# georgegrosu1/torch-admm-deconv

Measured on AMD Instinct MI355X. Metric: ADMM iterations/sec, batch-64 1024x1024x3, 50 iters; rel-L2 vs CPU ref, higher is better.
Workload: dtype f32

## Files before the change

torch-admm-deconv_amd/csrc/admm_capi.hip:

```cpp
#include <hip/hip_runtime.h>

#include <cstdlib>
#include <cstring>
#include <mutex>
#include <string>
#include <type_traits>
#include <vector>

#include "gcol_mm.hpp"
#include "knobs.hpp"
#include "mixed_capi.hpp"
#include "odd_capi.hpp"
#include "state_kernels.hpp"
#include "admm_tv.h"

using namespace admm;

namespace {

thread_local std::string g_err;

int fail(int code, const std::string& msg) {
    g_err = msg;
    return code;
// ... 319 lines not shown
            hipLaunchKernelGGL((k_iso_norm<N, true, false, true>), dim3(nb), dim3(G::NT), G::lds_bytes(), s, a);
        else if (first)
            hipLaunchKernelGGL((k_iso_norm<N, true, false, false>), dim3(nb), dim3(G::NT), G::lds_bytes(), s, a);
        else if (hist)
            hipLaunchKernelGGL((k_iso_norm<N, false, true, false>), dim3(nb), dim3(G::NT), G::lds_bytes(), s, a);
        else if (pl)
            hipLaunchKernelGGL((k_iso_norm<N, false, false, true>), dim3(nb), dim3(G::NT), G::lds_bytes(), s, a);
        else
            hipLaunchKernelGGL((k_iso_norm<N, false, false, false>), dim3(nb), dim3(G::NT), G::lds_bytes(), s, a);
        return launch_check("k_iso_norm");
    }
    template <bool ISO, bool LASTK, bool FIRSTK> static void bpa(const BwdArgs& a, unsigned nb, hipStream_t s) {
        using BG = BwdGeom<N>;
        hipLaunchKernelGGL((k_bwd_pass_a<N, ISO, LASTK, FIRSTK>), dim3(nb), dim3(BG::NT), BG::lds_bytes(), s, a);
    }
    static int bwd_pass_a(const BwdArgs& a, bool iso, bool lastk, bool firstk, hipStream_t s) {
        const unsigned nb = (unsigned)((a.nstrips + BwdGeom<N>::SG - 1) / BwdGeom<N>::SG);
        const int sel = (iso ? 4 : 0) | (lastk ? 2 : 0) | (firstk ? 1 : 0);
        switch (sel) {
            case 0: bpa<false, false, false>(a, nb, s); break;
            case 1: bpa<false, false, true>(a, nb, s); break;
            case 2: bpa<false, true, false>(a, nb, s); break;
            case 3: bpa<false, true, true>(a, nb, s); break;
            case 4: bpa<true, false, false>(a, nb, s); break;
            case 5: bpa<true, false, true>(a, nb, s); break;
            case 6: bpa<true, true, false>(a, nb, s); break;
            default: bpa<true, true, true>(a, nb, s); break;
        }
        return launch_check("k_bwd_pass_a");
    }
    static int bwd_iso_q(const BwdIsoArgs& a, bool lastk, hipStream_t s) {
        const unsigned nb = blocks(a.nitems);
        if (lastk)
            hipLaunchKernelGGL((k_bwd_iso_q<N, true>), dim3(nb), dim3(G::NT), G::lds_bytes(), s, a);
        else
            hipLaunchKernelGGL((k_bwd_iso_q<N, false>), dim3(nb), dim3(G::NT), G::lds_bytes(), s, a);
        return launch_check("k_bwd_iso_q");
    }
};

template <class F> int with_row(int N, F&& f) {
    switch (N) {
        case 8: return f(RowOps<8>{});
        case 16: return f(RowOps<16>{});
        case 32: return f(RowOps<32>{});
        case 64: return f(RowOps<64>{});
        case 128: return f(RowOps<128>{});
        case 256: return f(RowOps<256>{});
        case 512: return f(RowOps<512>{});
        case 1024: return f(RowOps<1024>{});
        default: return fail(ADMM_TV_EUNSUPPORTED, "unsupported W");
    }
}

template <class F> int with_col(int H, F&& f) {
    switch (H) {
        case 16: return f(std::integral_constant<int, 16>{});
        case 32: return f(std::integral_constant<int, 32>{});
        case 64: return f(std::integral_constant<int, 64>{});
        case 128: return f(std::integral_constant<int, 128>{});
        case 256: return f(std::integral_constant<int, 256>{});
        case 512: return f(std::integral_constant<int, 512>{});
        case 1024: return f(std::integral_constant<int, 1024>{});
        case 2048: return f(std::integral_constant<int, 2048>{});
        case 4096: return f(std::integral_constant<int, 4096>{});
        default: return fail(ADMM_TV_EUNSUPPORTED, "unsupported H");
    }
}

int col_e(int H) { return H >= 1024 ? 16 : H >= 64 ? 8 : 4; }

int passb_order(int H) { return std::max(1, std::min(64, env_int("ADMM_PASSB_GROUP", H >= 1024 ? 2 : 1))); }

int passb_gp(int H, int P, int ppm) {
    (void)H;
    int g = env_int("ADMM_PASSB_GP", 1);
    g = std::max(1, std::min(g, 64));
    while (g > 1 && (ppm % g)) --g;
    (void)P;
    return g;
}

template <int H, int C> int pass_b_hc(const cf* spec, cf* out, const float* fcT, const cf* mT, const cf* twH, int N,
                                      int P, int mode, int ppm, hipStream_t s) {
    using G = ColGeom<H, C>;
    const int colblocks = N / C;
    const int gp = passb_gp(H, P, ppm);
    const dim3 grid((unsigned)((long long)((P + gp - 1) / gp) * colblocks));
    const int order = gp > 1 ? 1 : passb_order(H);
    const int fpack = mode == 0 && env_int("ADMM_PASSB_FPACK", 1) ? 1 : 0;
    const int pmode = env_int("ADMM_PASSB_PMODE", 2);
    if (mode == 0) {
        if (int e = set_lds(k_pass_b<H, C, 0>, G::lds_bytes())) return e;
        hipLaunchKernelGGL((k_pass_b<H, C, 0>), grid, dim3(G::NT), G::lds_bytes(), s, spec, out, fcT, mT, twH, N, colblocks, ppm,
                           order, fpack, gp, P, pmode);
    } else if (mode == 1) {
        if (int e = set_lds(k_pass_b<H, C, 1>, G::lds_bytes())) return e;
        hipLaunchKernelGGL((k_pass_b<H, C, 1>), grid, dim3(G::NT), G::lds_bytes(), s, spec, out, fcT, mT, twH, N, colblocks, ppm,
                           order, fpack, gp, P, pmode);
    } else {
        if (int e = set_lds(k_pass_b<H, C, 2>, G::lds_bytes())) return e;
        hipLaunchKernelGGL((k_pass_b<H, C, 2>), grid, dim3(G::NT), G::lds_bytes(), s, spec, out, fcT, mT, twH, N, colblocks, ppm,
                           order, fpack, gp, P, pmode);
    }
    return launch_check("k_pass_b");
}

template <int H> int pass_b_h(const cf* spec, cf* out, const float* fcT, const cf* mT, const cf* twH, int N, int P,
                              int mode, int ppm, hipStream_t s) {
    constexpr int L = ColGeom<H, 1>::L;
    if constexpr (L <= 64) {
        if (mode == 0 && N >= 16 && env_int("ADMM_PASSB_PAIR", H <= 512 ? 1 : 0)) {
            using G = ColGeom<H, 8>;
            const int colblocks = N / 16;
            if (int e = set_lds(k_pass_b2<H, 8>, G::lds_bytes())) return e;
            hipLaunchKernelGGL((k_pass_b2<H, 8>), dim3((unsigned)((long long)P * colblocks)), dim3(G::NT), G::lds_bytes(),
                               s, spec, out, fcT, twH, N, colblocks, ppm, passb_order(H), env_int("ADMM_PASSB_FPACK", 1) ? 1 : 0);
            return launch_check("k_pass_b2");
        }
        int C = env_int("ADMM_PASSB_C", 8);
        if (C > N) C = N;
        if (C >= 16) return pass_b_hc<H, 16>(spec, out, fcT, mT, twH, N, P, mode, ppm, s);
        return pass_b_hc<H, 8>(spec, out, fcT, mT, twH, N, P, mode, ppm, s);
    } else if constexpr (L == 128) {
        return pass_b_hc<H, 8>(spec, out, fcT, mT, twH, N, P, mode, ppm, s);
    } else {
        return pass_b_hc<H, 4>(spec, out, fcT, mT, twH, N, P, mode, ppm, s);
    }
}

int pass_b_oop(int H, const cf* spec, cf* out, const float* fcT, const cf* mT, const cf* twH, int N, int P, int mode,
               hipStream_t s, int ppm = 0) {
    if (ppm <= 0) ppm = P;
    return with_col(H, [&](auto h) { return pass_b_h<decltype(h)::value>(spec, out, fcT, mT, twH, N, P, mode, ppm, s); });
}

int pass_b(int H, cf* spec, const float* fcT, const cf* mT, const cf* twH, int N, int P, int mode, hipStream_t s,
           int ppm = 0) {
    return pass_b_oop(H, spec, spec, fcT, mT, twH, N, P, mode, s, ppm);
}

template <int H, int C> int xspec_hc(const cf* U, const cf* V, cf* part, const cf* twH, int N, int P, int ppg,
                                     hipStream_t s) {
    using G = ColGeom<H, C>;
    const int colblocks = N / C;
    const int groups = (P + ppg - 1) / ppg;
    if (int e = set_lds(k_xspec<H, C, true>, G::lds_bytes())) return e;
    if (int e = set_lds(k_xspec<H, C, false>, G::lds_bytes())) return e;
    hipLaunchKernelGGL((k_xspec<H, C, true>), dim3(groups), dim3(G::NT), G::lds_bytes(), s, U, V, part, twH, N,
                       colblocks, P, ppg);
    if (colblocks > 1)
        hipLaunchKernelGGL((k_xspec<H, C, false>), dim3(groups * (colblocks - 1)), dim3(G::NT), G::lds_bytes(), s, U,
                           V, part, twH, N, colblocks, P, ppg);
    return launch_check("k_xspec");
}
template <int H> int xspec_h(const cf* U, const cf* V, cf* part, const cf* twH, int N, int P, int ppg, hipStream_t s) {
    constexpr int L = ColGeom<H, 1>::L;
    if constexpr (L <= 64) return xspec_hc<H, 8>(U, V, part, twH, N, P, ppg, s);
    else if constexpr (L == 128) return xspec_hc<H, 8>(U, V, part, twH, N, P, ppg, s);
    else return xspec_hc<H, 4>(U, V, part, twH, N, P, ppg, s);
}
int xspec(int H, const cf* U, const cf* V, cf* part, const cf* twH, int N, int P, int ppg, hipStream_t s) {
    return with_col(H, [&](auto h) { return xspec_h<decltype(h)::value>(U, V, part, twH, N, P, ppg, s); });
}

int grouped_train_check(const admm_tv_desc& d) {
    if (d.groups > 1 && !supported_hw(d.H, d.W))
        return fail(ADMM_TV_EUNSUPPORTED, "grouped training needs power-of-two H, W: one call per module");
    return 0;
}

int validate(const admm_tv_desc* d) {
    if (!d) return fail(ADMM_TV_EINVAL, "null descriptor");
    const bool empty_ok = d->iso && d->allreduce && d->B >= 0 && d->C >= 0;
    if ((empty_ok ? (d->B < 0 || d->C < 0) : (d->B <= 0 || d->C <= 0)) || d->H <= 0 || d->W <= 0 || d->maxit < 0 ||
        d->kh < 0 || d->kw < 0 || d->groups < 0)
        return fail(ADMM_TV_EINVAL, "invalid sizes or maxit");
    if (d->kh != d->kw) return fail(ADMM_TV_ENONSQUARE, "non-square PSF (the reference's H_t swaps H/W pads)");
    if (is_f64(*d) ? !f64_hw(d->H, d->W) : (!supported_hw(d->H, d->W) && !generic_hw(d->H, d->W)))
        return fail(ADMM_TV_EUNSUPPORTED, "unsupported H, W (admm_tv_supported / admm_tv_supported_f64: up to 65,536)");
    if (is_f64(*d) && d->groups > 1) return fail(ADMM_TV_EUNSUPPORTED, "groups > 1: fp32 only");
    if (d->kh > d->H || d->kw > d->W) return fail(ADMM_TV_EKERNEL, "PSF larger than the image");
    if (d->groups > 1 && ((!supported_hw(d->H, d->W) && !mixed_hw(d->H, d->W)) || (d->flags & ADMM_TV_FLAG_PSF_GRAD)))
        return fail(ADMM_TV_EUNSUPPORTED, "groups > 1 needs power-of-two or smooth H, W and no PSF gradient");
    return 0;
}

double spectra_scale(int H, int W) {
    return (supported_hw(H, W) ? 0.5 : 1.0) / ((double)H * (double)W);
}

template <class T>
int setup(const admm_tv_desc& d, const Layout& Lo, void* ws, const T* kern, const T* rho, hipStream_t s) {
    using C = cx_t<T>;
    ProfScope ps(3, s);
    const int H = (int)d.H, W = (int)d.W, N = W / 2, k = d.kh;
    const int nt = 256;
    hipLaunchKernelGGL(k_tables<C>, dim3((std::max(H, W) + nt - 1) / nt), dim3(nt), 0, s, at<C>(ws, Lo.twW),
                       at<C>(ws, Lo.twH), at<double2>(ws, Lo.twHd), H, W);
    if (int e = launch_check("k_tables")) return e;
    if (Lo.gen && !std::is_same<T, double>::value) {
        for (int dim = 0; dim < 2; ++dim) {
            const GPlan pl = make_plan(dim == 0 ? W : H);
            if (pl.ntab == 0) continue;
            hipLaunchKernelGGL(k_blue_tables, dim3((3 * 1024 * 64 + nt - 1) / nt), dim3(nt), 0, s,
                               at<cf>(ws, dim == 0 ? Lo.twW : Lo.twH), pl);
            if (int e = launch_check("k_blue_tables")) return e;
        }
    }
    if (k > 0) {
        const int n = k * (N + 1);
        hipLaunchKernelGGL(k_psf_rows<T>, dim3((n + nt - 1) / nt), dim3(nt), 0, s, kern, at<double2>(ws, Lo.G), k, N, W);
        if (int e = launch_check("k_psf_rows")) return e;
    }
    const int n = (N + 1) * H;
    if (rho) {
        for (int g = 0; g < ngroups_of(d); ++g) {
// ... 918 lines not shown
    const int ns = std::max(1, std::min(kMaxAux + 1, env_setting("ADMM_GEN_STREAMS", 2)));
    const std::vector<long long> parts = gen_parts(P, H, ns);
    const bool glb = make_plan(H, kF64<T>).glb || make_plan(W, kF64<T>).glb;
    if (!d.iso && !train && parts.size() > 1 && !glb && cap == hipStreamCaptureStatusNone) {
        int dev = 0;
        HIPCHK(hipGetDevice(&dev));
        std::vector<hipStream_t> aux;
        for (size_t i = 1; i < parts.size(); ++i) {
            hipStream_t x = aux_stream(s, dev, (int)i - 1);
            if (!x) return fail(ADMM_TV_EHIP, "auxiliary stream");
            aux.push_back(x);
        }
        ForkJoin fj(s, aux);
        if (fj.err != hipSuccess) return fail(ADMM_TV_EHIP, std::string("fork: ") + hipGetErrorString(fj.err));
        int e = 0;
        for (size_t i = 0; i < parts.size() && !e; ++i) {
            const long long p1 = i + 1 < parts.size() ? parts[i + 1] : P;
            e = solve_planes(parts[i], p1 - parts[i], i == 0 ? s : aux[i - 1]);
        }
        const hipError_t je = fj.finish();
        if (e) return e;
        if (je != hipSuccess) return fail(ADMM_TV_EHIP, std::string("join: ") + hipGetErrorString(je));
    } else {
        if (int e = solve_planes(0, P, s)) return e;
    }
    if constexpr (!kF64<T>) {
        if (sout) {
            const int ui = (d.maxit - 1) & 1;
            const bool none = d.maxit == 1 && !sin;
            return state_export(d, Lo, ws, out, none ? nullptr : u[2 * ui], none ? nullptr : u[2 * ui + 1], *sio->out, lam,
                                rho, 0, s);
        }
    }
    return 0;
}

long long mixed_slots(int N) {
    static std::mutex mu;
    static std::vector<std::pair<std::pair<int, int>, long long>> cache;
    int dev = 0;
    if (hipGetDevice(&dev) != hipSuccess) return 512;
    std::lock_guard<std::mutex> lk(mu);
    for (const auto& c : cache)
        if (c.first.first == dev && c.first.second == N) return c.second;
    long long slots = 0;
    int cus = 0;
    if (hipDeviceGetAttribute(&cus, hipDeviceAttributeMultiprocessorCount, dev) == hipSuccess)
        slots = (long long)cus * std::max(1, admm_mixed::pass_a_blocks_per_cu(N));
    if (slots <= 0) return 512;
    cache.push_back({{dev, N}, slots});
    return slots;
}
int strip_rows_mixed(int H, long long rows, int N, long long slots = 0) {
    if (const int e = env_int("ADMM_MIXED_R", 0); e > 0 && H % e == 0) return e;
    const int sg = 256 / std::max(1, admm_mixed::row_lanes(N));
    if (slots <= 0) slots = mixed_slots(N);
    int best = 1;
    double best_t = 1e300;
    for (int R = 1; R <= 32 && R <= H; ++R) {
        if (H % R) continue;
        const long long strips = rows / R;
        const long long blocks = (strips + sg - 1) / sg;
        const double t = (double)((blocks + slots - 1) / slots) * (R + 1);
        if (t < best_t - 1e-9 || (t < best_t + 1e-9 && R > best)) {
            best_t = t;
            best = R;
        }
    }
    return best;
}

struct FusedOps {
    const admm_tv_desc& d;
    const Layout& Lo;
    void* const ws;
    const int H, N;
    cf *const twW, *const twH;
    FusedOps(const admm_tv_desc& d_, const Layout& L, void* w)
        : d(d_), Lo(L), ws(w), H((int)d_.H), N((int)d_.W / 2), twW(at<cf>(w, L.twW)), twH(at<cf>(w, L.twH)) {}
};

struct Pow2Ops : FusedOps {
    static constexpr bool kPsfGrad = true;
    float* const fcT;
    cf* const mT;
    const bool coop;
    const int rev;
    const bool pf;
    Pow2Ops(const admm_tv_desc& d_, const Layout& L, void* w)
        : FusedOps(d_, L, w), fcT(at<float>(w, L.fcT)), mT(at<cf>(w, L.mT)),
          coop(env_int("ADMM_PASSA_COOP", 1) != 0), rev(env_int("ADMM_PASSA_REV", 0)),
          pf(env_int("ADMM_PASSA_PF", 1) != 0) {}
    int modules_per_pass(int G) const { return G; }
    bool lane_paired(bool train) const { return !train && env_int("ADMM_PL", (d.iso || d.W < 1024) ? 1 : 0) != 0; }
    int row_lanes() const {
        int L = 0;
        with_row(N, [&](auto ops) { return L = decltype(ops)::G::L; });
        return L;
    }
    int strip(long long rows, bool aniso_fwd) const { return strip_rows(H, N, rows, aniso_fwd, coop && !rev); }
    int r2c(const float* img, cf* spec, long long rows, hipStream_t s, bool pl = false) const {
        return with_row(N, [&](auto ops) { return decltype(ops)::r2c(img, spec, twW, rows, s, pl); });
    }
    int c2r(const cf* spec, float* img, long long rows, hipStream_t s) const {
        return with_row(N, [&](auto ops) { return decltype(ops)::c2r(spec, img, twW, rows, s); });
    }
    int col(const cf* in, cf* out, long long np, long long ppm, int , hipStream_t s) const {
        return pass_b_oop(H, in, out, fcT, mT, twH, N, (int)np, 0, s, (int)ppm);
    }
    int xspec(const cf* U, const cf* V, cf* part, long long P, int ppg, bool , hipStream_t s) const {
        return ::xspec(H, U, V, part, twH, N, (int)P, ppg, s);
    }
    int iso_norm(const IsoArgs& a, bool first, bool hist, hipStream_t s, bool pl) const {
        return with_row(N, [&](auto ops) { return decltype(ops)::iso_norm(a, first, hist, s, pl); });
    }
    int pass_a(const PassAArgs& a, bool iso, bool first, bool hist, hipStream_t s, bool pl) const {
        return with_row(N, [&](auto ops) { return decltype(ops)::pass_a(a, iso, first, hist, s, pl, coop, pf); });
    }
    int bwd_iso_q(const BwdIsoArgs& a, bool lastk, hipStream_t s) const {
        return with_row(N, [&](auto ops) { return decltype(ops)::bwd_iso_q(a, lastk, s); });
    }
    int bwd_pass_a(const BwdArgs& a, bool iso, bool lastk, bool firstk, hipStream_t s) const {
        return with_row(N, [&](auto ops) { return decltype(ops)::bwd_pass_a(a, iso, lastk, firstk, s); });
    }
    int make_b(const float* xin, float* bb, cf* spec, bool pl, hipStream_t s) const {
        if (d.kh > 0) return psf_transpose_into(d, Lo, ws, xin, bb, spec, 1, s, pl);
        return with_row(N, [&](auto ops) { return decltype(ops)::pair(xin, bb, d.B * d.C * H, s); });
    }
    int apply_ht_t(const float* bbar, float* gxin, cf* spec, hipStream_t s) const {
        return psf_transpose_into(d, Lo, ws, bbar, gxin, spec, 2, s);
    }
};

struct MixedOps : FusedOps {
    static constexpr bool kPsfGrad = true;
    const float* const fcM;
    static constexpr int rev = 0;
    MixedOps(const admm_tv_desc& d_, const Layout& L, void* w) : FusedOps(d_, L, w), fcM(at<float>(w, L.fcM)) {}
    int modules_per_pass(int) const { return 1; }
    bool lane_paired(bool) const { return false; }
    int row_lanes() const { return 0; }
    int strip(long long rows, bool) const { return strip_rows_mixed(H, rows, N); }
    int r2c(const float* img, cf* spec, long long rows, hipStream_t s, bool = false) const {
        return hip_code(admm_mixed::r2c(N, img, spec, twW, rows, s), "k_row_r2c_m");
    }
    int c2r(const cf* spec, float* img, long long rows, hipStream_t s) const {
        return hip_code(admm_mixed::c2r(N, spec, img, twW, rows, s), "k_row_c2r_m");
    }
    int col(const cf* in, cf* out, long long np, long long, int g0, hipStream_t s) const {
        return hip_code(admm_mixed::pass_b(H, in, out, fcM + (size_t)g0 * (2 * N + 1) * H, twH, N, np, s), "k_pass_b_m");
    }
    int xspec(const cf* U, const cf* V, cf* part, long long P, int ppg, bool weighted, hipStream_t s) const {
        return hip_code(admm_mixed::xspec(H, U, V, part, twH, N, P, ppg, weighted ? 0.25f : 1.f, s), "k_xspec_m");
    }
    int iso_norm(const IsoArgs& a, bool first, bool hist, hipStream_t s, bool) const {
        return hip_code(admm_mixed::iso_norm(N, a, first, hist, s), "k_iso_norm_m");
    }
    int pass_a(const PassAArgs& a, bool iso, bool first, bool hist, hipStream_t s, bool) const {
        return hip_code(admm_mixed::pass_a(N, a, iso, first, hist, s), "k_pass_a_m");
    }
    int bwd_iso_q(const BwdIsoArgs& a, bool lastk, hipStream_t s) const {
        return hip_code(admm_mixed::bwd_iso_q(N, a, lastk, s), "k_bwd_iso_q_m");
    }
    int bwd_pass_a(const BwdArgs& a, bool iso, bool lastk, bool firstk, hipStream_t s) const {
        return hip_code(admm_mixed::bwd_pass_a(N, a, iso, lastk, firstk, s), "k_bwd_pass_a_m");
    }
    int make_b(const float* xin, float* bb, cf* spec, bool, hipStream_t s) const {
        const long long P = d.B * d.C;
        if (env_int("ADMM_MIXED_BGEN", 0)) return gapply<float>(xin, bb, spec, Lo, ws, d, 1, s);
        if (int e = r2c(xin, spec, P * H, s)) return e;
        if (int e = hip_code(admm_mixed::pass_b_cm(H, spec, at<cf>(ws, Lo.mM), twH, N, P, s), "k_pass_b_m<cm>")) return e;
        return c2r(spec, bb, P * H, s);
    }
    int apply_ht_t(const float* bbar, float* gxin, cf* spec, hipStream_t s) const {
        return gapply<float>(bbar, gxin, spec, Lo, ws, d, 2, s);
    }
};

template <class B>
int fused_forward(const B& be, const float* xin, const float* lam, const float* rho, float* out, void* hist,
                  hipStream_t s, const StateIO* sio = nullptr) {
    const admm_tv_desc& d = be.d;
    const Layout& Lo = be.Lo;
    void* ws = be.ws;
    const int H = be.H, N = be.N, W = (int)d.W, G = ngroups_of(d);
    const long long Pm = d.B * d.C;
    cf* spec[2] = {at<cf>(ws, Lo.spec[0]), at<cf>(ws, Lo.spec[1])};
    float* u[4] = {at<float>(ws, Lo.u[0]), at<float>(ws, Lo.u[1]), at<float>(ws, Lo.u[2]), at<float>(ws, Lo.u[3])};
    const bool train = hist != nullptr;
    const HistView<float> hv(d, hist);
    const bool keep_t = B::kPsfGrad && train && hv.h.keep_t;
    const bool pl = be.lane_paired(train);
    const float* bimg = xin;
    if (d.kh > 0 || pl) {
        ProfScope ps(3, s);
        float* bb = at<float>(ws, Lo.b);
        if (int e = be.make_b(xin, bb, spec[0], pl, s)) return e;
        bimg = bb;
    }
    const int ng = be.modules_per_pass(G);
    const long long np = ng * Pm, rows = np * H;
    const int gpm = Lo.ngroups / G;
    const int R = be.strip(rows, !d.iso && !train);
    const bool sin = sio && sio->in, sout = sio && sio->out;
    const int sl = pl ? be.row_lanes() : 0;
    for (int g0 = 0; g0 < G; g0 += ng) {
        const float* lamg = lam + g0;
        const float* rhog = rho + g0;
        float* outg = out + (size_t)g0 * Pm * H * W;
        for (int g = 0; g < ng; ++g) {
            ProfScope ps(3, s);
            cf* t0 = (keep_t ? hv.r(1) : spec[0]) + (size_t)g * Pm * H * N;
            if (sin) {
                if (int e = state_import(d, *sio->in, bimg, outg, u[0], u[1], lamg, rhog, sl, s)) return e;
                if (int e = be.r2c(outg, t0, Pm * H, s, false)) return e;
                continue;
            }
            if (int e = be.r2c(bimg, t0, Pm * H, s, pl)) return e;
        }
        int cur = 0, uin = 0;
        for (int it = 1; it <= d.maxit; ++it) {
            {
                ProfScope ps(1, s);
                if (int e = be.col(keep_t ? hv.r(it) : spec[cur], spec[cur], np, Pm, g0, s)) return e;
            }
            if (it == d.maxit) {
                ProfScope ps(3, s);
                if (int e = be.c2r(spec[cur], outg, rows, s)) return e;
                if (sout) {
                    const bool none = d.maxit == 1 && !sin;
                    if (int e = state_export(d, Lo, ws, outg, none ? nullptr : u[2 * uin], none ? nullptr : u[2 * uin + 1],
                                             *sio->out, lamg, rhog, sl, s))
                        return e;
                }
                if (!train) break;
            }
            const bool first = (it == 1) && !sin;
            const float *uxi, *uyi, *nprev = nullptr;
            float *uxo, *uyo;
            if (train) {
                uxi = first ? nullptr : hv.a(it - 1, 0);
                uyi = first ? nullptr : hv.a(it - 1, 1);
                uxo = hv.a(it, 0);
                uyo = hv.a(it, 1);
                if (d.iso && !first) nprev = hv.n(it - 1);
            } else {
                uxi = u[2 * uin];
                uyi = u[2 * uin + 1];
                uxo = u[2 * (1 - uin)];
                uyo = u[2 * (1 - uin) + 1];
                if (it == d.maxit - 1 && !sout) uxo = uyo = nullptr;
            }
            const float* nsq = nullptr;
            if (d.iso) {
                ProfScope ps(2, s);
                float* nout = train ? hv.n(it) : at<float>(ws, Lo.nsq);
                IsoArgs ia{spec[cur], uxi, uyi, nprev, lamg, rhog, at<float>(ws, Lo.part), be.twW, (int)np, H, Lo.ppg,
                           (long long)ng * gpm * H, Pm};
                if (int e = be.iso_norm(ia, first, train, s, pl)) return e;
                const long long n4 = 2LL * H * W / 4;
                for (int g = 0; g < ng; ++g) {
                    hipLaunchKernelGGL(k_iso_reduce, dim3((unsigned)((n4 + 255) / 256)), dim3(256), 0, s,
                                       at<float4>(ws, Lo.part) + (size_t)g * gpm * n4,
                                       reinterpret_cast<float4*>(nout) + (size_t)g * n4, gpm, n4);
                    if (int e = launch_check("k_iso_reduce")) return e;
                }
                allreduce(d, nout, (size_t)ng * 2 * H * W, s);
                nsq = nout;
            }
            {
                ProfScope ps(0, s);
                cf* tout = (keep_t && it < d.maxit) ? hv.r(it + 1) : spec[1 - cur];
                PassAArgs pa{spec[cur], tout, bimg, uxi, uyi, uxo, uyo, nsq, nprev, lamg, rhog, be.twW, H, R, rows / R, Pm,
                             be.rev};
                if (int e = be.pass_a(pa, d.iso != 0, first, train, s, pl)) return e;
            }
            cur = 1 - cur;
            uin = 1 - uin;
        }
    }
    return 0;
}

int run_forward(const admm_tv_desc& d, const float* xin, const float* kern, const float* lam, const float* rho,
                float* out, void* ws, size_t ws_bytes, void* hist, hipStream_t s) {
    const Layout Lo = make_layout(d);
    if (int e = check_workspace(ws, ws_bytes, Lo.total)) return e;
    if (Lo.tr && !hist && d.maxit > 0) {
        const long long P = d.B * d.C;
        const int H = (int)d.H, W = (int)d.W;
        float* xT = at<float>(ws, Lo.xT);
        float* oT = at<float>(ws, Lo.oT);
        float* kT = d.kh > 0 ? at<float>(ws, Lo.kT) : nullptr;
        {
            ProfScope ps(3, s);
            hipError_t e = admm_odd::transpose(xin, xT, H, W, P, s);
            if (e == hipSuccess && kT) e = admm_odd::transpose(kern, kT, d.kh, d.kw, 1, s);
            if (e != hipSuccess) return fail(ADMM_TV_EHIP, std::string("k_transpose: ") + hipGetErrorString(e));
        }
        const admm_tv_desc dT = transposed(d);
        if (int e = run_forward(dT, xT, kT, lam, rho, oT, at<char>(ws, Lo.tws), ws_bytes - Lo.tws, nullptr, s)) return e;
        ProfScope ps(3, s);
        const hipError_t e = admm_odd::transpose(oT, out, W, H, P, s);
        return e == hipSuccess ? 0 : fail(ADMM_TV_EHIP, std::string("k_transpose: ") + hipGetErrorString(e));
    }
// ... 622 lines not shown
```

torch-admm-deconv_amd/csrc/admm_kernels.hpp:

```cpp
#pragma once
#include "fft_core.hpp"

namespace admm {

template <int N, class Cfg = RowCfg<N>> struct RowXf {
    static constexpr int E = Cfg::E;
    static constexpr int L = N / E;
    static constexpr int W = 2 * N;
    static_assert(L <= 64, "row transforms keep one row inside one wave");

    __device__ __forceinline__ static void partner(const cf (&v)[E], cf (&p)[E], int t) {
        const int src = (L - t) & (L - 1);
#pragma unroll
        for (int j = 0; j < E; ++j) {
            float a = __shfl(v[E - 1 - j].x, src, L);
            float b = __shfl(v[E - 1 - j].y, src, L);
            p[j] = (t == 0) ? v[(E - j) & (E - 1)] : mkc(a, b);
        }
    }

    template <int SYNC = 0>
    __device__ __forceinline__ static void c2r(cf (&v)[E], const RowBuf& buf, const cf* __restrict__ tw, int t) {
        cf p[E];
        partner(v, p, t);
// ... 223 lines not shown
                                                 const cf* __restrict__ twW_g, long long rows) {
    using G = RowKernelGeom<N>;
    constexpr int E = G::E, L = G::L;
    extern __shared__ __attribute__((aligned(16))) unsigned char smem[];
    cf* tw = reinterpret_cast<cf*>(smem);
    load_tw(tw, twW_g, G::W);
    __syncthreads();
    const int sgl = threadIdx.x / L, t = threadIdx.x % L;
    const long long row = (long long)blockIdx.x * G::SG + sgl;
    if (row >= rows) return;
    RowBuf buf{tw + G::W + sgl * RowBuf::slots(N)};
    const cf* src = spec + row * N;
    cf v[E];
#pragma unroll
    for (int j = 0; j < E; ++j) v[j] = src[t + L * j];
    RowXf<N>::c2r(v, buf, tw, t);
    cf* dst = reinterpret_cast<cf*>(img + row * G::W);
    st_row<E, L, PL, false>(dst, t, v);
}

template <int N>
__global__ void __launch_bounds__(256) k_row_pair(const float* __restrict__ img, float* __restrict__ out, long long rows) {
    using G = RowKernelGeom<N>;
    constexpr int E = G::E, L = G::L;
    const int sgl = threadIdx.x / L, t = threadIdx.x % L;
    const long long row = (long long)blockIdx.x * G::SG + sgl;
    if (row >= rows) return;
    cf v[E];
    ld_row<E, L, false, true>(reinterpret_cast<const cf*>(img + row * G::W), t, v);
    st_row<E, L, true, false>(reinterpret_cast<cf*>(out + row * G::W), t, v);
}

constexpr int pb_minw(int nt, size_t lds) {
    return (nt / 64 * ((160 * 1024) / lds >= 2 ? 2 : 1) + 3) / 4 > 4 ? 4
                                                                      : (nt / 64 * ((160 * 1024) / lds >= 2 ? 2 : 1) + 3) / 4;
}

template <int H, int C> struct ColGeom {
    static constexpr int E = RowCfg<H>::E, L = H / E, NT = C * L;
    static constexpr int SYNC = 1;
    static constexpr size_t lds_bytes() { return sizeof(cf) * (H + (size_t)H * C); }
};

static __global__ void k_fc_pack(const float* __restrict__ fcT, float* __restrict__ fcP, int H, int N, int E) {
    const int i = blockIdx.x * blockDim.x + threadIdx.x;
    if (i >= (N + 1) * H) return;
    const int L = H / E, kx = i / H, r = i % H, t = r / E, j = r % E;
    fcP[i] = fcT[(size_t)kx * H + t + L * j];
}

__device__ __forceinline__ unsigned xcd_remap(unsigned b, unsigned nb) {
    const unsigned x = b & 7u, i = b >> 3, q = nb >> 3, r = nb & 7u;
    return (x < r ? x * (q + 1) : r * (q + 1) + (x - r) * q) + i;
}

__device__ __forceinline__ unsigned xcd_pairs(unsigned b, unsigned nb) {
    if ((b | 15u) >= nb) return b;
    const unsigned x = b & 7u, s = b >> 3;
    return 2u * (8u * (s >> 1) + x) + (s & 1u);
}

__device__ __forceinline__ void pb_tile(unsigned lb, int colblocks, int order, bool pairs, int& p, int& cb) {
    const unsigned P = gridDim.x / (unsigned)colblocks, G = order > 1 ? (unsigned)order : 1u;
    const unsigned per = G * (unsigned)colblocks, grp = lb / per;
    if (G == 1 || (pairs && (colblocks & 1)) || (grp + 1) * G > P) {
        p = (int)(lb / (unsigned)colblocks);
        cb = (int)(lb % (unsigned)colblocks);
        return;
    }
    const unsigned rem = lb % per;
    if (pairs) {
        const unsigned r = rem >> 1;
        p = (int)(grp * G + r % G);
        cb = (int)(2 * (r / G) + (rem & 1u));
    } else {
        p = (int)(grp * G + rem % G);
        cb = (int)(rem / G);
    }
}

#ifndef ADMM_PASSB_MHOIST
#define ADMM_PASSB_MHOIST 1
#endif
template <int H, int C, int MODE>
__global__ void __launch_bounds__(C * (H / RowCfg<H>::E), pb_minw(C * (H / RowCfg<H>::E), sizeof(cf) * (H + (size_t)H * C)))
    k_pass_b(const cf* spec_in, cf* spec_out, const float* __restrict__ fcT, const cf* __restrict__ mT,
             const cf* __restrict__ twH_g, int N, int colblocks, int ppm, int order, int fpack, int gp, int P,
             int pmode) {
    using G = ColGeom<H, C>;
    constexpr int E = G::E, L = G::L;
    extern __shared__ __attribute__((aligned(16))) unsigned char smem[];
    cf* tw = reinterpret_cast<cf*>(smem);
    cf* data = tw + H;
    load_tw(tw, twH_g, H);
    const int tid = threadIdx.x;
    const int c = tid % C, t = tid / C;
    const unsigned rb = (pmode >> 1) == 1 ? xcd_remap(blockIdx.x, gridDim.x)
                        : (pmode >> 1) == 2 ? xcd_pairs(blockIdx.x, gridDim.x) : blockIdx.x;
    int pg, cb;
    pb_tile(rb, colblocks, order, true, pg, cb);
    if (pmode & 1) pg = (int)(gridDim.x / (unsigned)colblocks) - 1 - pg;
    const int col = cb * C + c;
    const int p0 = pg * gp;
    if (MODE == 0) fcT += (size_t)(p0 / ppm) * (N + 1) * H;
    const int voff = (t * N + col) * (int)sizeof(cf);
    const int sstep = L * N * (int)sizeof(cf);
    using MT = typename std::conditional<MODE == 0, float, cf>::type;
    MT m[E];
    auto load_m = [&]() {
        if (MODE == 0 && fpack) {
            const float* fcP = fcT + (size_t)(P / ppm) * (N + 1) * H;
            const float4* qq = reinterpret_cast<const float4*>(fcP + ((size_t)col * L + t) * E);
    #pragma unroll
            for (int j = 0; j < E / 4; ++j) {
                const float4 f = qq[j];
                if constexpr (MODE == 0) {
                    m[4 * j] = f.x;
                    m[4 * j + 1] = f.y;
                    m[4 * j + 2] = f.z;
                    m[4 * j + 3] = f.w;
                }
            }
        } else {
            const rsrc_t rm = MODE == 0 ? make_rsrc(fcT, (unsigned)((size_t)(N + 1) * H * sizeof(float)))
                                        : make_rsrc(mT, (unsigned)((size_t)(N + 1) * H * sizeof(cf)));
            const int mo = (col * H + t) * (int)sizeof(MT);
    #pragma unroll
            for (int j = 0; j < E; ++j) {
                if constexpr (MODE == 0) m[j] = bload_f(rm, mo, j * L * (int)sizeof(float));
                else if constexpr (MODE == 1) m[j] = bload_cf(rm, mo, j * L * (int)sizeof(cf));
                else m[j] = cconj(bload_cf(rm, mo, j * L * (int)sizeof(cf)));
            }
        }
    };
    if (ADMM_PASSB_MHOIST) load_m();
#pragma clang loop unroll(disable)
    for (int q = 0; q < gp; ++q) {
        const int p = p0 + q;
        if (p >= P) break;
        ColBuf<C> buf{data + c};
        const rsrc_t rs = make_rsrc(spec_in + (size_t)p * H * N, (unsigned)((size_t)H * N * sizeof(cf)));
        const rsrc_t ro = make_rsrc(spec_out + (size_t)p * H * N, (unsigned)((size_t)H * N * sizeof(cf)));
        cf v[E];
#pragma unroll
        for (int j = 0; j < E; ++j) v[j] = bload_cf<(ADMM_NT & 8) ? 2 : 0>(rs, voff, j * sstep);
        if (!ADMM_PASSB_MHOIST) load_m();
        __syncthreads();
        fft<H, L, -1, 1, 1>(v, buf, tw, t);
        if (cb == 0) {
            __syncthreads();
#pragma unroll
            for (int j = 0; j < E; ++j) buf.at(t + L * j) = v[j];
            __syncthreads();
            if (col == 0) {
#pragma unroll
                for (int j = 0; j < E; ++j) {
                    const int ky = t + L * j;
                    const cf qv = cconj(buf.at((H - ky) & (H - 1)));
                    if constexpr (MODE == 0) {
                        const float f0 = m[j], fn = fcT[(size_t)N * H + ky];
                        const float a = 0.5f * (f0 + fn), b = 0.5f * (f0 - fn);
                        v[j] = mkc(fmaf(a, v[j].x, b * qv.x), fmaf(a, v[j].y, b * qv.y));
                    } else {
                        const cf m0 = m[j], mn = MODE == 1 ? mT[(size_t)N * H + ky] : cconj(mT[(size_t)N * H + ky]);
                        const cf a = mkc(0.5f * (m0.x + mn.x), 0.5f * (m0.y + mn.y));
                        const cf b = mkc(0.5f * (m0.x - mn.x), 0.5f * (m0.y - mn.y));
                        v[j] = cadd(cmul(v[j], a), cmul(qv, b));
                    }
                }
            }
        }
        if (col != 0) {
#pragma unroll
            for (int j = 0; j < E; ++j) {
                if constexpr (MODE == 0) v[j] = cscale(v[j], m[j]);
                else v[j] = cmul(v[j], m[j]);
            }
        }
        fft<H, L, +1, 1, 1>(v, buf, tw, t);
#pragma unroll
        for (int j = 0; j < E; ++j) bstore_cf<(ADMM_NT & 4) ? 2 : 0>(ro, voff, j * sstep, v[j]);
    }
}

#ifndef PASSB2_MINW
#define PASSB2_MINW 4
#endif
__device__ __forceinline__ float4 bload_f4(rsrc_t r, int voff, int soff) {
    return __builtin_bit_cast(float4, __builtin_amdgcn_raw_buffer_load_b128(r, voff, soff, 0));
}
__device__ __forceinline__ void bstore_f4(rsrc_t r, int voff, int soff, float4 v) {
    typedef decltype(__builtin_amdgcn_raw_buffer_load_b128(r, 0, 0, 0)) V4;
    __builtin_amdgcn_raw_buffer_store_b128(__builtin_bit_cast(V4, v), r, voff, soff, 0);
}

template <int H, int CP>
__global__ void __launch_bounds__(CP * (H / RowCfg<H>::E), PASSB2_MINW)
    k_pass_b2(const cf* spec_in, cf* spec_out, const float* __restrict__ fcT, const cf* __restrict__ twH_g, int N,
              int colblocks, int ppm, int order, int fpack) {
    using G = ColGeom<H, CP>;
    constexpr int E = G::E, L = G::L;
    extern __shared__ __attribute__((aligned(16))) unsigned char smem[];
    cf* tw = reinterpret_cast<cf*>(smem);
    cf* data = tw + H;
    load_tw(tw, twH_g, H);
    const int tid = threadIdx.x;
    const int cp = tid % CP, t = tid / CP;
    int p, cb;
    pb_tile(xcd_remap(blockIdx.x, gridDim.x), colblocks, order, false, p, cb);
    const int col = cb * 2 * CP + 2 * cp;
    fcT += (size_t)(p / ppm) * (N + 1) * H;
    const rsrc_t rs = make_rsrc(spec_in + (size_t)p * H * N, (unsigned)((size_t)H * N * sizeof(cf)));
    const rsrc_t ro = make_rsrc(spec_out + (size_t)p * H * N, (unsigned)((size_t)H * N * sizeof(cf)));
    const int voff = (t * N + col) * (int)sizeof(cf);
    const int sstep = L * N * (int)sizeof(cf);
    cf v0[E], v1[E];
#pragma unroll
    for (int j = 0; j < E; ++j) {
        const float4 q = bload_f4(rs, voff, j * sstep);
        v0[j] = mkc(q.x, q.y);
        v1[j] = mkc(q.z, q.w);
    }
    const rsrc_t rm = make_rsrc(fcT, (unsigned)((size_t)(N + 1) * H * sizeof(float)));
    const int mo = (col * H + t) * (int)sizeof(float);
    const float* fcP = fcT + (size_t)(gridDim.x / colblocks / ppm) * (N + 1) * H;
    auto packed = [&](int c, float (&m)[E]) {
        const float4* q = reinterpret_cast<const float4*>(fcP + ((size_t)c * L + t) * E);
#pragma unroll
        for (int j = 0; j < E / 4; ++j) {
            const float4 f = q[j];
            m[4 * j] = f.x;
            m[4 * j + 1] = f.y;
            m[4 * j + 2] = f.z;
            m[4 * j + 3] = f.w;
        }
    };
    float m0[E], m1[E];
    if (fpack) {
        packed(col, m0);
    } else {
#pragma unroll
        for (int j = 0; j < E; ++j) m0[j] = bload_f(rm, mo, j * L * (int)sizeof(float));
    }
    __syncthreads();
    ColBuf<CP> buf{data + cp};
    fft<H, L, -1, 1, 1>(v0, buf, tw, t);
    if (cb == 0) {
        __syncthreads();
#pragma unroll
        for (int j = 0; j < E; ++j) buf.at(t + L * j) = v0[j];
        __syncthreads();
        if (col == 0) {
#pragma unroll
            for (int j = 0; j < E; ++j) {
                const int ky = t + L * j;
                const cf q = cconj(buf.at((H - ky) & (H - 1)));
                const float f0 = m0[j], fn = fcT[(size_t)N * H + ky];
                const float a = 0.5f * (f0 + fn), b = 0.5f * (f0 - fn);
                v0[j] = mkc(fmaf(a, v0[j].x, b * q.x), fmaf(a, v0[j].y, b * q.y));
            }
        }
// ... 555 lines not shown
```

Baseline: 762.2.

## Reuse half-transformed setup spectrum to skip first-iteration init column pass

```diff
diff --git a/torch-admm-deconv_amd/csrc/admm_capi.hip b/torch-admm-deconv_amd/csrc/admm_capi.hip
--- a/torch-admm-deconv_amd/csrc/admm_capi.hip
+++ b/torch-admm-deconv_amd/csrc/admm_capi.hip
@@ -425,32 +425,29 @@
 }
 
 template <int H, int C> int pass_b_hc(const cf* spec, cf* out, const float* fcT, const cf* mT, const cf* twH, int N,
-                                      int P, int mode, int ppm, hipStream_t s) {
+                                      int P, int mode, int ppm, hipStream_t s, int inmod, cf* outb) {
     using G = ColGeom<H, C>;
     const int colblocks = N / C;
     const int gp = passb_gp(H, P, ppm);
     const dim3 grid((unsigned)((long long)((P + gp - 1) / gp) * colblocks));
     const int order = gp > 1 ? 1 : passb_order(H);
-    const int fpack = mode == 0 && env_int("ADMM_PASSB_FPACK", 1) ? 1 : 0;
+    const int fpack = (mode == 0 || mode == 4) && env_int("ADMM_PASSB_FPACK", 1) ? 1 : 0;
+    const float s1scale = 4.f * (float)N;
     const int pmode = env_int("ADMM_PASSB_PMODE", 2);
-    if (mode == 0) {
-        if (int e = set_lds(k_pass_b<H, C, 0>, G::lds_bytes())) return e;
-        hipLaunchKernelGGL((k_pass_b<H, C, 0>), grid, dim3(G::NT), G::lds_bytes(), s, spec, out, fcT, mT, twH, N, colblocks, ppm,
-                           order, fpack, gp, P, pmode);
-    } else if (mode == 1) {
-        if (int e = set_lds(k_pass_b<H, C, 1>, G::lds_bytes())) return e;
-        hipLaunchKernelGGL((k_pass_b<H, C, 1>), grid, dim3(G::NT), G::lds_bytes(), s, spec, out, fcT, mT, twH, N, colblocks, ppm,
-                           order, fpack, gp, P, pmode);
-    } else {
-        if (int e = set_lds(k_pass_b<H, C, 2>, G::lds_bytes())) return e;
-        hipLaunchKernelGGL((k_pass_b<H, C, 2>), grid, dim3(G::NT), G::lds_bytes(), s, spec, out, fcT, mT, twH, N, colblocks, ppm,
-                           order, fpack, gp, P, pmode);
-    }
-    return launch_check("k_pass_b");
+    auto launch = [&](auto kern) {
+        if (int e = set_lds(kern, G::lds_bytes())) return e;
+        hipLaunchKernelGGL(kern, grid, dim3(G::NT), G::lds_bytes(), s, spec, out, fcT, mT, twH, N, colblocks, ppm, order,
+                           fpack, gp, P, pmode, inmod > 0 ? inmod : P, s1scale, outb);
+        return launch_check("k_pass_b");
+    };
+    if (mode == 0) return launch(k_pass_b<H, C, 0>);
+    if (mode == 1) return launch(k_pass_b<H, C, 1>);
+    if (mode == 2) return launch(k_pass_b<H, C, 2>);
+    return launch(k_pass_b<H, C, 4>);
 }
 
 template <int H> int pass_b_h(const cf* spec, cf* out, const float* fcT, const cf* mT, const cf* twH, int N, int P,
-                              int mode, int ppm, hipStream_t s) {
+                              int mode, int ppm, hipStream_t s, int inmod, cf* outb) {
     constexpr int L = ColGeom<H, 1>::L;
     if constexpr (L <= 64) {
         if (mode == 0 && N >= 16 && env_int("ADMM_PASSB_PAIR", H <= 512 ? 1 : 0)) {
@@ -463,19 +460,21 @@
         }
         int C = env_int("ADMM_PASSB_C", 8);
         if (C > N) C = N;
-        if (C >= 16) return pass_b_hc<H, 16>(spec, out, fcT, mT, twH, N, P, mode, ppm, s);
-        return pass_b_hc<H, 8>(spec, out, fcT, mT, twH, N, P, mode, ppm, s);
+        if (C >= 16) return pass_b_hc<H, 16>(spec, out, fcT, mT, twH, N, P, mode, ppm, s, inmod, outb);
+        return pass_b_hc<H, 8>(spec, out, fcT, mT, twH, N, P, mode, ppm, s, inmod, outb);
     } else if constexpr (L == 128) {
-        return pass_b_hc<H, 8>(spec, out, fcT, mT, twH, N, P, mode, ppm, s);
+        return pass_b_hc<H, 8>(spec, out, fcT, mT, twH, N, P, mode, ppm, s, inmod, outb);
     } else {
-        return pass_b_hc<H, 4>(spec, out, fcT, mT, twH, N, P, mode, ppm, s);
+        return pass_b_hc<H, 4>(spec, out, fcT, mT, twH, N, P, mode, ppm, s, inmod, outb);
     }
 }
 
 int pass_b_oop(int H, const cf* spec, cf* out, const float* fcT, const cf* mT, const cf* twH, int N, int P, int mode,
-               hipStream_t s, int ppm = 0) {
+               hipStream_t s, int ppm = 0, int inmod = 0, cf* outb = nullptr) {
     if (ppm <= 0) ppm = P;
-    return with_col(H, [&](auto h) { return pass_b_h<decltype(h)::value>(spec, out, fcT, mT, twH, N, P, mode, ppm, s); });
+    return with_col(H, [&](auto h) {
+        return pass_b_h<decltype(h)::value>(spec, out, fcT, mT, twH, N, P, mode, ppm, s, inmod, outb);
+    });
 }
 
 int pass_b(int H, cf* spec, const float* fcT, const cf* mT, const cf* twH, int N, int P, int mode, hipStream_t s,
@@ -1560,15 +1559,29 @@
 
 struct Pow2Ops : FusedOps {
     static constexpr bool kPsfGrad = true;
+    static constexpr bool kSetupS1 = true;
     float* const fcT;
     cf* const mT;
     const bool coop;
     const int rev;
     const bool pf;
+    const int setup;
+    const bool setup_iso;
     Pow2Ops(const admm_tv_desc& d_, const Layout& L, void* w)
         : FusedOps(d_, L, w), fcT(at<float>(w, L.fcT)), mT(at<cf>(w, L.mT)),
           coop(env_int("ADMM_PASSA_COOP", 1) != 0), rev(env_int("ADMM_PASSA_REV", 0)),
-          pf(env_int("ADMM_PASSA_PF", 1) != 0) {}
+          pf(env_int("ADMM_PASSA_PF", 1) != 0), setup(env_int("ADMM_SETUP_FUSED", 1)),
+          setup_iso(env_int("ADMM_SETUP_ISO", 0) != 0) {}
+    bool setup_s1() const { return d.kh > 0 && setup >= 1 && (!d.iso || setup_iso); }
+    int make_b_s1(const float* xin, float* bb, cf* spec, cf* s1, bool pl, hipStream_t s) const {
+        const long long Pm = d.B * d.C;
+        if (int e = r2c(xin, spec, Pm * H, s)) return e;
+        if (int e = pass_b_oop(H, spec, s1, fcT, mT, twH, N, (int)Pm, 1, s)) return e;
+        return with_row(N, [&](auto ops) { return decltype(ops)::c2r(s1, bb, twW, Pm * H, s, pl); });
+    }
+    int col_s1(const cf* s1, cf* out, cf* r1, long long np, long long ppm, hipStream_t s) const {
+        return pass_b_oop(H, s1, out, fcT, mT, twH, N, (int)np, 4, s, (int)ppm, (int)ppm, r1);
+    }
     int modules_per_pass(int G) const { return G; }
     bool lane_paired(bool train) const { return !train && env_int("ADMM_PL", (d.iso || d.W < 1024) ? 1 : 0) != 0; }
     int row_lanes() const {
@@ -1612,6 +1625,7 @@
 
 struct MixedOps : FusedOps {
     static constexpr bool kPsfGrad = true;
+    static constexpr bool kSetupS1 = false;
     const float* const fcM;
     static constexpr int rev = 0;
     MixedOps(const admm_tv_desc& d_, const Layout& L, void* w) : FusedOps(d_, L, w), fcM(at<float>(w, L.fcM)) {}
@@ -1669,24 +1683,30 @@
     const HistView<float> hv(d, hist);
     const bool keep_t = B::kPsfGrad && train && hv.h.keep_t;
     const bool pl = be.lane_paired(train);
+    const bool sin = sio && sio->in, sout = sio && sio->out;
+    bool s1 = false;
+    cf* const s1buf = spec[1];
+    if constexpr (B::kSetupS1) s1 = be.setup_s1() && !sin;
     const float* bimg = xin;
     if (d.kh > 0 || pl) {
         ProfScope ps(3, s);
         float* bb = at<float>(ws, Lo.b);
-        if (int e = be.make_b(xin, bb, spec[0], pl, s)) return e;
+        int e;
+        if constexpr (B::kSetupS1) e = s1 ? be.make_b_s1(xin, bb, spec[0], s1buf, pl, s) : be.make_b(xin, bb, spec[0], pl, s);
+        else e = be.make_b(xin, bb, spec[0], pl, s);
+        if (e) return e;
         bimg = bb;
     }
     const int ng = be.modules_per_pass(G);
     const long long np = ng * Pm, rows = np * H;
     const int gpm = Lo.ngroups / G;
     const int R = be.strip(rows, !d.iso && !train);
-    const bool sin = sio && sio->in, sout = sio && sio->out;
     const int sl = pl ? be.row_lanes() : 0;
     for (int g0 = 0; g0 < G; g0 += ng) {
         const float* lamg = lam + g0;
         const float* rhog = rho + g0;
         float* outg = out + (size_t)g0 * Pm * H * W;
-        for (int g = 0; g < ng; ++g) {
+        for (int g = 0; g < ng && !s1; ++g) {
             ProfScope ps(3, s);
             cf* t0 = (keep_t ? hv.r(1) : spec[0]) + (size_t)g * Pm * H * N;
             if (sin) {
@@ -1698,7 +1718,12 @@
         }
         int cur = 0, uin = 0;
         for (int it = 1; it <= d.maxit; ++it) {
-            {
+            if (it == 1 && s1) {
+                if constexpr (B::kSetupS1) {
+                    ProfScope ps(1, s);
+                    if (int e = be.col_s1(s1buf, spec[cur], keep_t ? hv.r(1) : nullptr, np, Pm, s)) return e;
+                }
+            } else {
                 ProfScope ps(1, s);
                 if (int e = be.col(keep_t ? hv.r(it) : spec[cur], spec[cur], np, Pm, g0, s)) return e;
             }
diff --git a/torch-admm-deconv_amd/csrc/admm_kernels.hpp b/torch-admm-deconv_amd/csrc/admm_kernels.hpp
--- a/torch-admm-deconv_amd/csrc/admm_kernels.hpp
+++ b/torch-admm-deconv_amd/csrc/admm_kernels.hpp
@@ -329,13 +329,16 @@
 #ifndef ADMM_PASSB_MHOIST
 #define ADMM_PASSB_MHOIST 1
 #endif
+template <int MM> using pb_mult_t = typename std::conditional<MM == 0, float, cf>::type;
+
 template <int H, int C, int MODE>
 __global__ void __launch_bounds__(C * (H / RowCfg<H>::E), pb_minw(C * (H / RowCfg<H>::E), sizeof(cf) * (H + (size_t)H * C)))
     k_pass_b(const cf* spec_in, cf* spec_out, const float* __restrict__ fcT, const cf* __restrict__ mT,
              const cf* __restrict__ twH_g, int N, int colblocks, int ppm, int order, int fpack, int gp, int P,
-             int pmode) {
+             int pmode, int inmod, float s1scale, cf* spec_b) {
     using G = ColGeom<H, C>;
     constexpr int E = G::E, L = G::L;
+    constexpr int M1 = MODE == 4 ? 0 : MODE;
     extern __shared__ __attribute__((aligned(16))) unsigned char smem[];
     cf* tw = reinterpret_cast<cf*>(smem);
     cf* data = tw + H;
@@ -349,81 +352,97 @@
     if (pmode & 1) pg = (int)(gridDim.x / (unsigned)colblocks) - 1 - pg;
     const int col = cb * C + c;
     const int p0 = pg * gp;
-    if (MODE == 0) fcT += (size_t)(p0 / ppm) * (N + 1) * H;
+    if (M1 == 0) fcT += (size_t)(p0 / ppm) * (N + 1) * H;
     const int voff = (t * N + col) * (int)sizeof(cf);
     const int sstep = L * N * (int)sizeof(cf);
-    using MT = typename std::conditional<MODE == 0, float, cf>::type;
-    MT m[E];
-    auto load_m = [&]() {
-        if (MODE == 0 && fpack) {
+    auto load_m = [&](auto mode, auto& mm) {
+        constexpr int MM = decltype(mode)::value;
+        using MT = pb_mult_t<MM>;
+        if (MM == 0 && fpack) {
             const float* fcP = fcT + (size_t)(P / ppm) * (N + 1) * H;
             const float4* qq = reinterpret_cast<const float4*>(fcP + ((size_t)col * L + t) * E);
     #pragma unroll
             for (int j = 0; j < E / 4; ++j) {
                 const float4 f = qq[j];
-                if constexpr (MODE == 0) {
-                    m[4 * j] = f.x;
-                    m[4 * j + 1] = f.y;
-                    m[4 * j + 2] = f.z;
-                    m[4 * j + 3] = f.w;
+                if constexpr (MM == 0) {
+                    mm[4 * j] = f.x;
+                    mm[4 * j + 1] = f.y;
+                    mm[4 * j + 2] = f.z;
+                    mm[4 * j + 3] = f.w;
                 }
             }
         } else {
-            const rsrc_t rm = MODE == 0 ? make_rsrc(fcT, (unsigned)((size_t)(N + 1) * H * sizeof(float)))
-                                        : make_rsrc(mT, (unsigned)((size_t)(N + 1) * H * sizeof(cf)));
+            const rsrc_t rm = MM == 0 ? make_rsrc(fcT, (unsigned)((size_t)(N + 1) * H * sizeof(float)))
+                                      : make_rsrc(mT, (unsigned)((size_t)(N + 1) * H * sizeof(cf)));
             const int mo = (col * H + t) * (int)sizeof(MT);
     #pragma unroll
             for (int j = 0; j < E; ++j) {
-                if constexpr (MODE == 0) m[j] = bload_f(rm, mo, j * L * (int)sizeof(float));
-                else if constexpr (MODE == 1) m[j] = bload_cf(rm, mo, j * L * (int)sizeof(cf));
-                else m[j] = cconj(bload_cf(rm, mo, j * L * (int)sizeof(cf)));
+                if constexpr (MM == 0) mm[j] = bload_f(rm, mo, j * L * (int)sizeof(float));
+                else if constexpr (MM == 1) mm[j] = bload_cf(rm, mo, j * L * (int)sizeof(cf));
+                else mm[j] = cconj(bload_cf(rm, mo, j * L * (int)sizeof(cf)));
             }
         }
     };
-    if (ADMM_PASSB_MHOIST) load_m();
+    auto mult = [&](auto mode, const auto& mm, cf(&v)[E], ColBuf<C>& buf) {
+        constexpr int MM = decltype(mode)::value;
+        if (cb == 0) {
+            __syncthreads();
+#pragma unroll
+            for (int j = 0; j < E; ++j) buf.at(t + L * j) = v[j];
+            __syncthreads();
+            if (col == 0) {
+#pragma unroll
+                for (int j = 0; j < E; ++j) {
+                    const int ky = t + L * j;
+                    const cf qv = cconj(buf.at((H - ky) & (H - 1)));
+                    if constexpr (MM == 0) {
+                        const float f0 = mm[j], fn = fcT[(size_t)N * H + ky];
+                        const float a = 0.5f * (f0 + fn), b = 0.5f * (f0 - fn);
+                        v[j] = mkc(fmaf(a, v[j].x, b * qv.x), fmaf(a, v[j].y, b * qv.y));
+                    } else {
+                        const cf m0 = mm[j], mn = MM == 1 ? mT[(size_t)N * H + ky] : cconj(mT[(size_t)N * H + ky]);
+                        const cf a = mkc(0.5f * (m0.x + mn.x), 0.5f * (m0.y + mn.y));
+                        const cf b = mkc(0.5f * (m0.x - mn.x), 0.5f * (m0.y - mn.y));
+                        v[j] = cadd(cmul(v[j], a), cmul(qv, b));
+                    }
+                }
+            }
+        }
+        if (col != 0) {
+#pragma unroll
+            for (int j = 0; j < E; ++j) {
+                if constexpr (MM == 0) v[j] = cscale(v[j], mm[j]);
+                else v[j] = cmul(v[j], mm[j]);
+            }
+        }
+    };
+    constexpr std::integral_constant<int, M1> m1{};
+    pb_mult_t<M1> m[E];
+    if (ADMM_PASSB_MHOIST) load_m(m1, m);
 #pragma clang loop unroll(disable)
     for (int q = 0; q < gp; ++q) {
         const int p = p0 + q;
         if (p >= P) break;
         ColBuf<C> buf{data + c};
-        const rsrc_t rs = make_rsrc(spec_in + (size_t)p * H * N, (unsigned)((size_t)H * N * sizeof(cf)));
+        const rsrc_t rs = make_rsrc(spec_in + (size_t)(MODE == 4 ? p % inmod : p) * H * N,
+                                    (unsigned)((size_t)H * N * sizeof(cf)));
         const rsrc_t ro = make_rsrc(spec_out + (size_t)p * H * N, (unsigned)((size_t)H * N * sizeof(cf)));
         cf v[E];
 #pragma unroll
         for (int j = 0; j < E; ++j) v[j] = bload_cf<(ADMM_NT & 8) ? 2 : 0>(rs, voff, j * sstep);
-        if (!ADMM_PASSB_MHOIST) load_m();
+        if constexpr (MODE == 4) {
+#pragma unroll
+            for (int j = 0; j < E; ++j) v[j] = cscale(v[j], s1scale);
+            if (spec_b) {
+                const rsrc_t rb1 = make_rsrc(spec_b + (size_t)p * H * N, (unsigned)((size_t)H * N * sizeof(cf)));
+#pragma unroll
+                for (int j = 0; j < E; ++j) bstore_cf<(ADMM_NT & 4) ? 2 : 0>(rb1, voff, j * sstep, v[j]);
+            }
+        }
+        if (!ADMM_PASSB_MHOIST) load_m(m1, m);
         __syncthreads();
         fft<H, L, -1, 1, 1>(v, buf, tw, t);
-        if (cb == 0) {
-            __syncthreads();
-#pragma unroll
-            for (int j = 0; j < E; ++j) buf.at(t + L * j) = v[j];
-            __syncthreads();
-            if (col == 0) {
-#pragma unroll
-                for (int j = 0; j < E; ++j) {
-                    const int ky = t + L * j;
-                    const cf qv = cconj(buf.at((H - ky) & (H - 1)));
-                    if constexpr (MODE == 0) {
-                        const float f0 = m[j], fn = fcT[(size_t)N * H + ky];
-                        const float a = 0.5f * (f0 + fn), b = 0.5f * (f0 - fn);
-                        v[j] = mkc(fmaf(a, v[j].x, b * qv.x), fmaf(a, v[j].y, b * qv.y));
-                    } else {
-                        const cf m0 = m[j], mn = MODE == 1 ? mT[(size_t)N * H + ky] : cconj(mT[(size_t)N * H + ky]);
-                        const cf a = mkc(0.5f * (m0.x + mn.x), 0.5f * (m0.y + mn.y));
-                        const cf b = mkc(0.5f * (m0.x - mn.x), 0.5f * (m0.y - mn.y));
-                        v[j] = cadd(cmul(v[j], a), cmul(qv, b));
-                    }
-                }
-            }
-        }
-        if (col != 0) {
-#pragma unroll
-            for (int j = 0; j < E; ++j) {
-                if constexpr (MODE == 0) v[j] = cscale(v[j], m[j]);
-                else v[j] = cmul(v[j], m[j]);
-            }
-        }
+        mult(m1, m, v, buf);
         fft<H, L, +1, 1, 1>(v, buf, tw, t);
 #pragma unroll
         for (int j = 0; j < E; ++j) bstore_cf<(ADMM_NT & 4) ? 2 : 0>(ro, voff, j * sstep, v[j]);
```

Measured after the change: 765.8 (median of 6 runs). No clear change (+0.5%).
